# Alex-McAvoy/Light-Graph-Convolutional-Recommendation-Algorithm-based-on-Hybrid-Spreading

Measured on AMD Instinct MI355X. Metric: propagation edges/sec + full-catalog top-K recs/sec, 1/2/4/8 MI355X, higher is better.
Workload: dtype f32; 1 GPU; c5-d64; users=1000000, items=1000000, interactions=100000000, directed_nnz=200000000, dim=64, layers=3, parallelism=row-shard x1 + RCCL all-gather per layer

## Files before the change

include/lgcnhs.h:

```cpp
#ifndef LGCNHS_H
#define LGCNHS_H

#include <stddef.h>
#include <stdint.h>

#ifdef __cplusplus
extern "C" {
#endif

typedef void *lg_stream_t;

enum lg_status {
  LG_OK = 0,
  LG_ERR_ARG = 1,
  LG_ERR_HIP = 2,
  LG_ERR_WORKSPACE = 3,
};

#define LG_ABI_VERSION 16
int lg_abi_version(void);
const char *lg_last_error(void);


int lg_csr_rowptr_from_sorted(const int64_t *keys, int64_t nnz, int64_t n_rows,
                              int64_t *rowptr, lg_stream_t stream);

int lg_gcn_norm_f32(const int64_t *rowptr, int64_t n_nodes, float *dis,
                    lg_stream_t stream);

int lg_gcn_edge_weight_f32(const int64_t *rowptr, const int32_t *src, const float *dis,
                           int64_t n_rows, int64_t row_offset, float *w,
                           lg_stream_t stream);

enum lg_acc_mode {
  LG_ACC_NONE = 0,
  LG_ACC_FIRST = 1,
  LG_ACC_MID = 2,
  LG_ACC_LAST = 3,
  LG_ACC_ONLY = 4,
};
int lg_spmm_layer_f32(const int64_t *rowptr, const int32_t *src, const float *dis,
                      const float *w, const float *x, float *y, const float *x0, float *acc,
// ... 39 lines not shown
                      lg_stream_t stream);
int lg_spmm_long_rows_f16(const int64_t *seg_beg, const int64_t *seg_end,
                          const int32_t *seg_node, int64_t n_seg, const int32_t *long_node,
                          const int64_t *seg_ptr, int64_t n_long, const int32_t *src,
                          const float *dis, const float *w, const void *xh, void *yh,
                          const float *x0, float *acc, float *out, int32_t dim,
                          int32_t acc_mode, float denom, float *partial, lg_stream_t stream);

size_t lg_score_topk_ws_bytes(int64_t n_users, int64_t n_items, int32_t dim, int32_t k,
                              int32_t n_splits);
int lg_score_topk_f32(const float *eu, const float *ei, int64_t n_users, int64_t n_items,
                      int32_t dim, const int64_t *ex_rowptr, const int32_t *ex_col,
                      float mask_value, int32_t k, int32_t n_splits, float *out_val,
                      int64_t *out_idx, void *ws, size_t ws_bytes, lg_stream_t stream);

size_t lg_score_topk_screened_ws_bytes(int64_t n_users, int64_t n_items, int32_t dim,
                                       int32_t k, int32_t n_splits);
int lg_score_topk_screened_f32(const float *eu, const float *ei, const void *eu_bf16,
                               const void *ei_bf16, const float *umarg, int64_t n_users,
                               int64_t n_items, int32_t dim, const int64_t *ex_rowptr,
                               const int32_t *ex_col, float mask_value, int32_t k,
                               int32_t n_splits, float *out_val, int64_t *out_idx, void *ws,
                               size_t ws_bytes, lg_stream_t stream);

int lg_score_dense_f32(const float *eu, const float *ei, int64_t n_users, int64_t n_items,
                       int32_t dim, const int64_t *ex_rowptr, const int32_t *ex_col,
                       float mask_value, float *G, int64_t ldg, lg_stream_t stream);


int lg_spread_general_f64(const int64_t *item_rowptr, const int32_t *item_users,
                          const int64_t *user_rowptr, const int32_t *user_items,
                          int64_t n_users, int64_t n_items, double *gW,
                          lg_stream_t stream);

size_t lg_spread_hybrid_ws_bytes(int64_t n_items, int64_t n_users);
int lg_spread_hybrid_f64(const int64_t *item_rowptr, const int32_t *item_users,
                         const int64_t *user_rowptr, const int32_t *user_items,
                         const double *k_item, int64_t n_users, int64_t n_items, double lambda,
                         double *W, void *ws, size_t ws_bytes, lg_stream_t stream);

int lg_hybrid_weight_f64(const double *gW, const double *k_item, int64_t n_items,
                         double lambda, int32_t transpose_gw, double *W,
                         lg_stream_t stream);

int lg_spread_resource_f64(const int64_t *user_rowptr, const int32_t *user_items,
                           const double *W, int64_t n_users, int64_t n_items, double *F,
// ... 84 lines not shown
```

light-graph-convolutional-recommendation-algorithm-based-on-hybrid-spreading_amd/csrc/topk.hip:

```cpp
#include <stdlib.h>

#include "common.h"

namespace lg {

typedef float f32x4 __attribute__((ext_vector_type(4)));

template <int Q>
__device__ __forceinline__ void load_piece(const float *__restrict__ p, float (&v)[Q]) {
  const float4 *p4 = reinterpret_cast<const float4 *>(p);
#pragma unroll
  for (int t = 0; t < Q / 4; ++t) {
    const float4 q = p4[t];
    v[4 * t + 0] = q.x;
    v[4 * t + 1] = q.y;
    v[4 * t + 2] = q.z;
    v[4 * t + 3] = q.w;
  }
}

typedef float f32x4v __attribute__((ext_vector_type(4)));

typedef unsigned u32x4v __attribute__((ext_vector_type(4)));
template <int D>
// ... 295 lines not shown
#define LG_RING_LA 5
#endif
#ifndef LG_RING_LAG
#define LG_RING_LAG 1
#endif
#ifndef LG_RING2_CAP
#define LG_RING2_CAP 112
#endif
#ifndef LG_RING2_NBUF
#define LG_RING2_NBUF 9
#endif
#ifndef LG_RING4_CAP
#define LG_RING4_CAP 160
#endif
#ifndef LG_RING4_NBUF
#define LG_RING4_NBUF 4
#endif
#ifndef LG_RING4_LA
#define LG_RING4_LA 2
#endif
#ifndef LG_RING4_W
#define LG_RING4_W 8
#endif
#ifndef LG_RING_NG
#define LG_RING_NG 2
#endif
#ifndef LG_RING_W
#define LG_RING_W (16 / LG_RING_NG)
#endif

constexpr int ring_chunk_bytes(int D, int W) {
  if (W == 8 || W == 4) return D >= 64 || W >= 8 ? 8192 : 4096;
  for (int m = 1; m < 64; ++m) {
    const int cb = 1024 * W * m;
    if (cb >= 4096 && (cb / (2 * D)) % 16 == 0) return cb;
  }
  return 0;
}

template <int D, int NG, int WAVES, int M, int CAP, int NBUF, int LA, int LAG, bool SEEDP,
          bool GL = false>
__global__ __launch_bounds__(64 * WAVES) void k_topk_ring(
    const float *__restrict__ eu, const float *__restrict__ ei, const __bf16 *__restrict__ eub,
    const __bf16 *__restrict__ eib, const float *__restrict__ umarg, int64_t n_users,
    int64_t n_items, const int64_t *__restrict__ ex_rowptr,
    const int32_t *__restrict__ ex_col, float mask_value, int k, int n_splits,
    int64_t items_per_split, float *__restrict__ out_val, int64_t *__restrict__ out_idx,
    float *__restrict__ part_val, int32_t *__restrict__ part_idx,
    const float *__restrict__ seed_val, uint2 *__restrict__ gl_list) {
  static_assert(M == 1 || M == 2 || M == 4, "list slabs");
  static_assert(GL ? (CAP <= 64 && CAP > 16) : (CAP <= 64 * M && CAP > 32 * M), "list capacity");
  constexpr int CAPG = 64 * M;
  constexpr int Q = D / 4;
  constexpr int S = D / 32;
  constexpr int CB = ring_chunk_bytes(D, WAVES);
  constexpr int CI = CB / (2 * D), TPC = CI / 16, PR = D / 8, RB = 2 * D;
  constexpr int PPT = CB / 16 / (64 * WAVES);
  static_assert(PPT >= 1 && CI * PR == 64 * WAVES * PPT, "whole DMA pieces per thread");
  static_assert(LAG >= 1 && LA > LAG && NBUF > LA, "ring shape");
  constexpr int TPC_S = TPC < 4 ? TPC : 4;
  constexpr int NCLS = 16 * TPC_S;
  constexpr int R = M == 1 ? (NCLS >= 64 ? 1 : 2) : 4;
  __shared__ uint32_t lk[WAVES][NG][16][SEEDP ? 1 : CAP];
  __shared__ uint16_t lt[WAVES][NG][16][SEEDP ? 1 : CAP];
  __shared__ int exs[WAVES][64];
  __shared__ __attribute__((aligned(16))) char frs[NBUF][CI * RB];
  __shared__ uint32_t prog[WAVES];

  const int wave = threadIdx.x / 64;
  const int lane = lane_id();
  const int ul = lane & 15;
  const int gq = lane >> 4;
  const int64_t tile = blockIdx.x / n_splits;
  const int split = blockIdx.x % n_splits;
  const int64_t ubase = (tile * WAVES + wave) * (16 * NG);
  const int64_t i0 = (int64_t)split * items_per_split;
  int64_t i1 = i0 + items_per_split;
  if (i1 > n_items) i1 = n_items;
  const int n_valid = i1 > i0 ? (int)(i1 - i0) : 0;
  const int n_t = (n_valid + 15) / 16;

  bf16x8 ub[NG][S];
  float marg[NG];
  bool uvalid[NG];
  int64_t ex_pos[NG], ex_hi[NG];
// ... 555 lines not shown
      if constexpr (SEEDP) {
        seed_chunk(c, acc);
        LG_CLK1(9, t_scr);
        continue;
      }
      uint32_t gm = test_chunk(acc);
      LG_CLK1(9, t_scr);
#ifdef LG_SCREEN_PROBE
      asm volatile("" ::"s"(gm));
      gm = 0;
#endif
      if (gm != 0) process_hits(c, acc, gm);
    }
    asm volatile("s_waitcnt vmcnt(0)" ::: "memory");
  }

  wave_sync();
  if constexpr (SEEDP) {
    constexpr int NV = TPC_S * R * 4;
#pragma unroll
    for (int g = 0; g < NG; ++g) {
      const int64_t user = ubase + g * 16 + ul;
      int E = 0;
      if (ex_rowptr && user < n_users) {
        const int64_t e0 = ex_rowptr[user], e1 = ex_rowptr[user + 1];
        E = (int)(lower_bound_i32(ex_col, e0, e1, (int32_t)i1) -
                  lower_bound_i32(ex_col, e0, e1, (int32_t)i0));
      }
      const int need = k + E;
      uint32_t o[NV];
#pragma unroll
      for (int tt = 0; tt < TPC_S; ++tt)
#pragma unroll
        for (int l = 0; l < R; ++l)
#pragma unroll
          for (int r = 0; r < 4; ++r) {
            const float x = cmax[g][tt][l][r];
            o[(tt * R + l) * 4 + r] = ford(x);
          }
      uint32_t T = 0u;
#pragma unroll 1
      for (int b = 31; b >= 0; --b) {
        const uint32_t c = T | (1u << b);
        int n = 0;
#pragma unroll
        for (int j = 0; j < NV; ++j) n += o[j] >= c ? 1 : 0;
        n += __shfl_xor(n, 16);
        n += __shfl_xor(n, 32);
        if (n >= need) T = c;
      }
// ... 243 lines not shown
#endif
#ifndef LG_GL4_NG
#define LG_GL4_NG 1
#endif
#ifndef LG_GL_NG
#define LG_GL_NG 2
#endif
#ifndef LG_TOPK_LDS_LISTS
#define LG_TOPK_LDS_LISTS 0
#endif
static int screen_slab_m(int k) {
  if (LG_TOPK_LDS_LISTS) return 0;
  if (k <= 32) return LG_TOPK_GL32 ? 2 : 0;
  return k <= 64 ? 2 : 4;
}

template <int D>
static void dispatch_topk_screen(int M, bool seedp, const float *eu, const float *ei,
                                 const __bf16 *eub, const __bf16 *eib, const float *umarg,
                                 int64_t n_users, int64_t n_items, const int64_t *ex_rowptr,
                                 const int32_t *ex_col, float mask_value, int k, int n_splits,
                                 int64_t items_per_split, float *out_val, int64_t *out_idx,
                                 float *part_val, int32_t *part_idx, const float *seed_val,
                                 uint2 *gl_list, hipStream_t stream) {
#define LG_RING_LAUNCH(NG, W, MM, CAP, NBUF, LA, LAG, SEEDP, GLM)                             \
  {                                                                                           \
    const int64_t upb = (int64_t)(W) * (NG) * 16;                                             \
    const int64_t tiles = (n_users + upb - 1) / upb;                                          \
    k_topk_ring<D, NG, W, MM, CAP, NBUF, LA, LAG, SEEDP, GLM>                                 \
        <<<dim3((unsigned)(tiles * n_splits)), dim3(64 * (W)), 0, stream>>>(                  \
            eu, ei, eub, eib, umarg, n_users, n_items, ex_rowptr, ex_col, mask_value, k,      \
            n_splits, items_per_split, out_val, out_idx, part_val, part_idx, seed_val,        \
            gl_list);                                                                         \
  }
  const int gm = seedp ? 0 : screen_slab_m(k);
  if (gm == 2) {
    LG_RING_LAUNCH(LG_GL_NG, 8, 2, LG_GL_CAP, LG_GL_NBUF, LG_GL_LA, 1, false, true)
  } else if (gm == 4) {
    LG_RING_LAUNCH((D <= 64 ? LG_GL4_NG : LG_GL_NG), 8, 4, LG_GL_CAP, LG_GL_NBUF, LG_GL_LA, 1,
                   false, true)
  } else if (M == 1 && seedp) {
    LG_RING_LAUNCH(LG_RING_NG, LG_RING_W, 1, LG_RING_CAP, LG_RING_NBUF, LG_RING_LA,
                   LG_RING_LAG, true, false)
  } else if (M == 1) {
    LG_RING_LAUNCH(LG_RING_NG, LG_RING_W, 1, LG_RING_CAP, LG_RING_NBUF, LG_RING_LA,
                   LG_RING_LAG, false, false)
  } else if (M == 2 && seedp) {
    LG_RING_LAUNCH(1, 8, 2, LG_RING2_CAP, LG_RING2_NBUF, LG_RING_LA, LG_RING_LAG, true, false)
  } else if (M == 2) {
    if (LG_TOPK_LDS_LISTS)
      LG_RING_LAUNCH(1, 8, 2, LG_RING2_CAP, LG_RING2_NBUF, LG_RING_LA, LG_RING_LAG, false, false)
  } else if (seedp) {
    LG_RING_LAUNCH(LG_SEED4_NG, 8, 4, 160, LG_SEED4_NBUF, LG_SEED4_LA, 1, true, false)
  } else if constexpr (D > 64) {
    if (LG_TOPK_LDS_LISTS) LG_RING_LAUNCH(1, 8, 4, 160, 4, 2, 1, false, false)
  } else {
// ... 4 lines not shown
}

static int cap_m(int k) { return k <= 32 ? 1 : (k <= 64 ? 2 : 4); }

static size_t screened_part_bytes(int64_t n_users, int k, int ns) {
  return ns > 1 ? (size_t)ns * (size_t)n_users * (size_t)k * (sizeof(float) + sizeof(int32_t))
                : 0;
}
static size_t screened_slab_bytes(int64_t n_users, int k, int ns) {
  return (size_t)ns * (size_t)n_users * 64 * (size_t)screen_slab_m(k) * sizeof(uint2);
}

static int64_t split_len(int64_t n_items, int n_splits) {
  int64_t per = (n_items + n_splits - 1) / n_splits;
  per = (per + 15) / 16 * 16;
  return per < 16 ? 16 : per;
}

static int screened_splits(int64_t n_items, int n_splits) {
  const int64_t need = (n_items + ((int64_t)1 << (kTileBits + 4)) - 1) >> (kTileBits + 4);
  return n_splits > need ? n_splits : (int)need;
}

}

using namespace lg;

extern "C" size_t lg_score_topk_ws_bytes(int64_t n_users, int64_t n_items, int32_t dim,
                                         int32_t k, int32_t n_splits) {
  (void)dim;
  if (n_items > 0 && n_splits >= 1) n_splits = screened_splits(n_items, n_splits);
  if (n_splits <= 1 || n_users <= 0 || k <= 0) return 0;
  return (size_t)n_splits * (size_t)n_users * (size_t)k * (sizeof(float) + sizeof(int32_t));
}

extern "C" size_t lg_score_topk_screened_ws_bytes(int64_t n_users, int64_t n_items,
                                                  int32_t dim, int32_t k, int32_t n_splits) {
  (void)dim;
  if (n_users <= 0 || n_items <= 0 || n_items >= 0x7fffffff || k < 1 || k > 128 ||
      n_splits < 1)
    return 0;
  const int64_t per = split_len(n_items, screened_splits(n_items, n_splits));
  const int ns = (int)((n_items + per - 1) / per);
  return screened_part_bytes(n_users, k, ns) + screened_slab_bytes(n_users, k, ns);
}

// ... 24 lines not shown
    part_val = (float *)ws;
    part_idx = (int32_t *)((char *)ws + (size_t)ns * n_users * k * sizeof(float));
  }
  hipStream_t s = (hipStream_t)stream;
  const int M = cap_m(k);
  if (topk_probe() == 2) ex_rowptr = nullptr, ex_col = nullptr;
  switch (dim) {
    case 32: dispatch_topk<32>(M, eu, ei, n_users, n_items, ex_rowptr, ex_col, mask_value, k, ns, per, out_val, out_idx, part_val, part_idx, s); break;
    case 64: dispatch_topk<64>(M, eu, ei, n_users, n_items, ex_rowptr, ex_col, mask_value, k, ns, per, out_val, out_idx, part_val, part_idx, s); break;
    default: dispatch_topk<128>(M, eu, ei, n_users, n_items, ex_rowptr, ex_col, mask_value, k, ns, per, out_val, out_idx, part_val, part_idx, s); break;
  }
  int st = launch_status("lg_score_topk_f32");
  if (st != LG_OK || ns == 1) return st;
  const unsigned blocks = (unsigned)((n_users + 3) / 4);
  if (k <= 64)
    k_topk_merge<2><<<dim3(blocks), dim3(256), 0, s>>>(part_val, part_idx, n_users, k, ns,
                                                        out_val, out_idx);
  else
    k_topk_merge<4><<<dim3(blocks), dim3(256), 0, s>>>(part_val, part_idx, n_users, k, ns,
                                                        out_val, out_idx);
  return launch_status("lg_score_topk_f32(merge)");
}

extern "C" int lg_score_topk_screened_f32(const float *eu, const float *ei, const void *eu_bf16,
                                          const void *ei_bf16, const float *umarg,
                                          int64_t n_users, int64_t n_items, int32_t dim,
                                          const int64_t *ex_rowptr, const int32_t *ex_col,
                                          float mask_value, int32_t k, int32_t n_splits,
                                          float *out_val, int64_t *out_idx, void *ws,
                                          size_t ws_bytes, lg_stream_t stream) {
  LG_REQUIRE(eu && ei && eu_bf16 && ei_bf16 && umarg && out_val && out_idx,
             "lg_score_topk_screened_f32: null pointer");
  LG_REQUIRE(n_users >= 0 && n_items > 0 && n_items < 0x7fffffff,
             "lg_score_topk_screened_f32: n_items must be in [1, 2^31-1)");
  LG_REQUIRE(dim == 32 || dim == 64 || dim == 128,
             "lg_score_topk_screened_f32: dim %d not in {32,64,128}", dim);
  LG_REQUIRE(k >= 1 && k <= 128, "lg_score_topk_screened_f32: k=%d not in [1,128]", k);
  LG_REQUIRE(n_splits >= 1 && n_splits <= 4096, "lg_score_topk_screened_f32: bad n_splits %d",
             n_splits);
  LG_REQUIRE(!ex_rowptr == !ex_col,
             "lg_score_topk_screened_f32: ex_rowptr/ex_col must both be set");
  LG_REQUIRE(((uintptr_t)eu_bf16 & 15) == 0 && ((uintptr_t)ei_bf16 & 15) == 0,
             "lg_score_topk_screened_f32: bf16 copies must be 16-byte aligned");
  if (n_users == 0) return LG_OK;
  const int64_t per = split_len(n_items, screened_splits(n_items, n_splits));
  const int ns = (int)((n_items + per - 1) / per);
  float *part_val = nullptr;
  int32_t *part_idx = nullptr;
  uint2 *gl_list = nullptr;
  {
    const size_t part = screened_part_bytes(n_users, k, ns);
    const size_t need = part + screened_slab_bytes(n_users, k, ns);
    if (need > 0 && (!ws || ws_bytes < need)) {
      set_error("lg_score_topk_screened_f32: workspace %zu < %zu bytes", ws_bytes, need);
      return LG_ERR_WORKSPACE;
    }
    if (ns > 1) {
      part_val = (float *)ws;
      part_idx = (int32_t *)((char *)ws + (size_t)ns * n_users * k * sizeof(float));
    }
    if (screen_slab_m(k)) gl_list = (uint2 *)((char *)ws + part);
  }
  hipStream_t s = (hipStream_t)stream;
  const int M = cap_m(k);
  const __bf16 *ub = (const __bf16 *)eu_bf16, *ib = (const __bf16 *)ei_bf16;
  auto pass = [&](bool seedp, int64_t n_it, int nsp, int64_t per_sp, const float *seed) {
    switch (dim) {
      case 32: dispatch_topk_screen<32>(M, seedp, eu, ei, ub, ib, umarg, n_users, n_it, ex_rowptr, ex_col, mask_value, k, nsp, per_sp, out_val, out_idx, part_val, part_idx, seed, gl_list, s); break;
      case 64: dispatch_topk_screen<64>(M, seedp, eu, ei, ub, ib, umarg, n_users, n_it, ex_rowptr, ex_col, mask_value, k, nsp, per_sp, out_val, out_idx, part_val, part_idx, seed, gl_list, s); break;
      default: dispatch_topk_screen<128>(M, seedp, eu, ei, ub, ib, umarg, n_users, n_it, ex_rowptr, ex_col, mask_value, k, nsp, per_sp, out_val, out_idx, part_val, part_idx, seed, gl_list, s); break;
    }
    int st = launch_status("lg_score_topk_screened_f32");
    if (st != LG_OK || nsp == 1) return st;
    if (seedp) {
      k_seed_combine<<<dim3((unsigned)((n_users + 255) / 256)), dim3(256), 0, s>>>(
          part_val, n_users, k, nsp, out_val);
      return launch_status("lg_score_topk_screened_f32(seeds)");
    }
    const unsigned blocks = (unsigned)((n_users + 3) / 4);
    if (k <= 64)
      k_topk_merge<2><<<dim3(blocks), dim3(256), 0, s>>>(part_val, part_idx, n_users, k, nsp,
                                                          out_val, out_idx);
    else
      k_topk_merge<4><<<dim3(blocks), dim3(256), 0, s>>>(part_val, part_idx, n_users, k, nsp,
                                                          out_val, out_idx);
    return launch_status("lg_score_topk_screened_f32(merge)");
  };
  const int64_t n_seed = n_items / (k > 32 ? LG_TOPK_SEED_DIV_HI : LG_TOPK_SEED_DIV) / 16 * 16;
  const bool seeded = lg_topk_seeding() && n_seed >= (int64_t)k * 64;
  if (seeded) {
    const int64_t per_s = split_len(n_seed, ns);
    const int ns_s = (int)((n_seed + per_s - 1) / per_s);
    const int st = pass(true, n_seed, ns_s, per_s, nullptr);
    if (st != LG_OK) return st;
  }
  return pass(false, n_items, ns, per, seeded ? out_val : nullptr);
}

extern "C" int lg_score_dense_f32(const float *eu, const float *ei, int64_t n_users,
                                  int64_t n_items, int32_t dim, const int64_t *ex_rowptr,
                                  const int32_t *ex_col, float mask_value, float *G,
                                  int64_t ldg, lg_stream_t stream) {
  LG_REQUIRE(eu && ei && G, "lg_score_dense_f32: null pointer");
  LG_REQUIRE(n_users >= 0 && n_items >= 0 && n_items < 0x7fffffff && ldg >= n_items,
             "lg_score_dense_f32: bad sizes");
  LG_REQUIRE(dim == 32 || dim == 64 || dim == 128, "lg_score_dense_f32: dim %d not in {32,64,128}",
             dim);
  LG_REQUIRE(!ex_rowptr == !ex_col, "lg_score_dense_f32: ex_rowptr/ex_col must both be set");
  if (n_users == 0 || n_items == 0) return LG_OK;
  const int64_t ipb = 1024;
  const int64_t chunks = (n_items + ipb - 1) / ipb;
  const int64_t ugrps = (n_users + 63) / 64;
  hipStream_t s = (hipStream_t)stream;
  dim3 grid((unsigned)(ugrps * chunks)), block(256);
  switch (dim) {
    case 32: k_score_dense<32><<<grid, block, 0, s>>>(eu, ei, n_users, n_items, ex_rowptr, ex_col, mask_value, G, ldg, ipb); break;
    case 64: k_score_dense<64><<<grid, block, 0, s>>>(eu, ei, n_users, n_items, ex_rowptr, ex_col, mask_value, G, ldg, ipb); break;
    default: k_score_dense<128><<<grid, block, 0, s>>>(eu, ei, n_users, n_items, ex_rowptr, ex_col, mask_value, G, ldg, ipb); break;
  }
// ... 13 lines not shown
```

light-graph-convolutional-recommendation-algorithm-based-on-hybrid-spreading_amd/lgcnhs/_native.py:

```python
from __future__ import annotations

import ctypes
import os
import threading

import torch

PKG_DIR = os.path.dirname(os.path.dirname(os.path.abspath(__file__)))
LIB_PATH = os.path.join(PKG_DIR, "lib", "liblgcnhs.so")
LIB_PATH = os.environ.get("LGCNHS_LIB_PATH") or LIB_PATH

LG_OK = 0
LG_ACC_NONE, LG_ACC_FIRST, LG_ACC_MID, LG_ACC_LAST, LG_ACC_ONLY = 0, 1, 2, 3, 4
LG_EXCL_DROP, LG_EXCL_NONE = 0, 1
ABI_VERSION = 16

_vp = ctypes.c_void_p
_i64 = ctypes.c_int64
_i32 = ctypes.c_int32
_f32 = ctypes.c_float
_f64 = ctypes.c_double
_sz = ctypes.c_size_t

SIGNATURES = {
    "lg_abi_version": (ctypes.c_int, []),
    "lg_last_error": (ctypes.c_char_p, []),
    "lg_csr_rowptr_from_sorted": (ctypes.c_int, [_vp, _i64, _i64, _vp, _vp]),
    "lg_gcn_norm_f32": (ctypes.c_int, [_vp, _i64, _vp, _vp]),
    "lg_gcn_edge_weight_f32": (ctypes.c_int, [_vp, _vp, _vp, _i64, _i64, _vp, _vp]),
    "lg_spmm_layer_f32": (
        ctypes.c_int,
        [_vp, _vp, _vp, _vp, _vp, _vp, _vp, _vp, _vp, _i64, _i64, _i32, _i32, _f32, _i64, _vp],
    ),
    "lg_spmm_layer_live_f32": (
        ctypes.c_int,
        [_vp, _vp, _vp, _vp, _vp, _vp, _vp, _vp, _vp, _i64, _i64, _i32, _i32, _f32, _i64, _vp,
         _vp],
    ),
# ... 13 lines not shown
         _f32, _vp, _vp, _vp],
    ),
    "lg_mark_neighbors_u8": (ctypes.c_int, [_vp, _vp, _i64, _vp, _vp, _vp]),
    "lg_rows_f32_to_f16": (ctypes.c_int, [_vp, _i64, _i32, _vp, _vp]),
    "lg_spmm_layer_f16": (
        ctypes.c_int,
        [_vp, _vp, _vp, _vp, _vp, _vp, _vp, _vp, _vp, _i64, _i64, _i32, _i32, _f32, _i64, _vp],
    ),
    "lg_spmm_long_rows_f16": (
        ctypes.c_int,
        [_vp, _vp, _vp, _i64, _vp, _vp, _i64, _vp, _vp, _vp, _vp, _vp, _vp, _vp, _vp, _i32, _i32,
         _f32, _vp, _vp],
    ),
    "lg_score_topk_ws_bytes": (_sz, [_i64, _i64, _i32, _i32, _i32]),
    "lg_score_topk_screened_ws_bytes": (_sz, [_i64, _i64, _i32, _i32, _i32]),
    "lg_score_topk_f32": (
        ctypes.c_int,
        [_vp, _vp, _i64, _i64, _i32, _vp, _vp, _f32, _i32, _i32, _vp, _vp, _vp, _sz, _vp],
    ),
    "lg_score_topk_screened_f32": (
        ctypes.c_int,
        [_vp, _vp, _vp, _vp, _vp, _i64, _i64, _i32, _vp, _vp, _f32, _i32, _i32, _vp, _vp, _vp,
         _sz, _vp],
    ),
    "lg_score_dense_f32": (
        ctypes.c_int,
        [_vp, _vp, _i64, _i64, _i32, _vp, _vp, _f32, _vp, _i64, _vp],
    ),
    "lg_spread_general_f64": (ctypes.c_int, [_vp, _vp, _vp, _vp, _i64, _i64, _vp, _vp]),
    "lg_hybrid_weight_f64": (ctypes.c_int, [_vp, _vp, _i64, _f64, _i32, _vp, _vp]),
    "lg_spread_hybrid_ws_bytes": (_sz, [_i64, _i64]),
    "lg_spread_hybrid_f64": (ctypes.c_int, [_vp, _vp, _vp, _vp, _vp, _i64, _i64, _f64, _vp, _vp,
                                            _sz, _vp]),
    "lg_spread_resource_f64": (ctypes.c_int, [_vp, _vp, _vp, _i64, _i64, _vp, _i64, _vp]),
    "lg_rows_topk_f64": (
        ctypes.c_int,
        [_vp, _i64, _i64, _i64, _vp, _vp, _i32, _vp, _vp, _i32, _i32, _vp, _vp, _vp],
    ),
    "lg_hybrid_recip_f64": (ctypes.c_int, [_vp, _i64, _f64, _vp, _vp, _vp]),
    "lg_inv_degree_f64": (ctypes.c_int, [_vp, _i64, _vp, _vp]),
    "lg_spread_group_cursor": (ctypes.c_int, [_vp, _vp, _vp, _i64, _i32, _i32, _i32, _i32, _vp,
                                              _vp, _vp, _vp, _vp]),
    "lg_spread_group_bound": (ctypes.c_int, [_vp, _vp, _i64, _vp, _i32, _vp, _vp]),
    "lg_spread_group_units": (ctypes.c_int, [_vp, _i64, _i32, _i32, _i32, _i32, _i64, _vp, _vp]),
    "lg_spread_group_rows_ws_bytes": (_sz, [_i64, _i32]),
    "lg_spread_group_rows_f64": (
# ... 116 lines not shown
```

light-graph-convolutional-recommendation-algorithm-based-on-hybrid-spreading_amd/lgcnhs/ops.py:

```python
from __future__ import annotations

import numpy as np
import torch

from . import _native as N
from .graph import Adjacency, RowSets

MASK_VALUE = float(-(1 << 10))


def _f32(t: torch.Tensor, name: str) -> torch.Tensor:
    N.require_gpu(t, name)
    if t.dtype != torch.float32:
        raise TypeError(f"{name} must be float32, got {t.dtype}")
    return t.contiguous()


def run_layer(rowptr, src, dis, w, x, y, x0, acc, out, n_rows: int, row_offset: int,
              mode: int, denom: float, plan=None, live=None, row_mask=None) -> None:
    dim = x.shape[1]
    thr = plan.threshold if (plan is not None and plan.n_long) else 0
    strm = N.stream_handle(x.device)
    half = x.dtype == torch.float16
    if half:
# ... 285 lines not shown
SCREEN_DEFAULT = True
SCREEN_MIN_WORK = {32: 6e8, 128: 1e9}


def screen_pays(n_users: int, n_items: int, k: int) -> bool:
    for kmax, work in SCREEN_MIN_WORK.items():
        if k <= kmax:
            return float(n_users) * float(n_items) >= work
    return False


def screen_margins(un: torch.Tensor, ue: torch.Tensor, inorm: torch.Tensor,
                   ierr: torch.Tensor, dim: int) -> torch.Tensor:
    I = inorm.max().double()
    DI = ierr.max().double()
    u, e = un.double(), ue.double()
    m = (e * I + (u + e) * DI + (2.01 * dim * 2.0 ** -24 + 2.0 ** -22) * u * I) \
        * (1.0 + 2.0 ** -20) + 1e-30
    m32 = m.float()
    return torch.where(m32.double() < m, torch.nextafter(m32, torch.full_like(m32, float("inf"))),
                       m32)


def score_topk(eu: torch.Tensor, ei: torch.Tensor, k: int, excl: RowSets | None = None,
               mask_value: float = MASK_VALUE, n_splits: int | None = None,
               screen: bool | None = None):
    eu, ei = _f32(eu, "eu"), _f32(ei, "ei")
    nu, d = eu.shape
    ni = ei.shape[0]
    if screen is None:
        screen = SCREEN_DEFAULT and screen_pays(nu, ni, k)
    if ei.shape[1] != d:
        raise ValueError("eu/ei dims differ")
    if excl is not None and excl.n_rows != nu:
        raise ValueError(f"exclusion rows {excl.n_rows} != users {nu}")
    ns = (_splits_for(nu, ni, k, _resident_blocks(eu.device, k, screen), screen, d)
          if n_splits is None else int(n_splits))
    ws_fn = (N.lib().lg_score_topk_screened_ws_bytes if screen and nu > 0
             else N.lib().lg_score_topk_ws_bytes)
    ws_bytes = ws_fn(nu, ni, d, k, ns)
    ws = torch.empty(max(ws_bytes, 1), dtype=torch.uint8, device=eu.device)
    val = torch.empty((nu, k), dtype=torch.float32, device=eu.device)
    idx = torch.empty((nu, k), dtype=torch.int64, device=eu.device)
    ex_rp = N.ptr(excl.rowptr if excl else None)
    ex_c = N.ptr(excl.col if excl else None)
    if screen and nu > 0:
        ub, un, ue = bound_operands(eu, with_err=True)
        ib, inorm, ierr = bound_operands(ei, with_err=True)
        umarg = screen_margins(un, ue, inorm, ierr, d)
        N.check(N.lib().lg_score_topk_screened_f32(
            N.ptr(eu), N.ptr(ei), N.ptr(ub), N.ptr(ib), N.ptr(umarg), nu, ni, d, ex_rp, ex_c,
            float(mask_value), int(k), ns, N.ptr(val), N.ptr(idx), N.ptr(ws), ws_bytes,
            N.stream_handle(eu.device)), "lg_score_topk_screened_f32")
        return val, idx
    N.check(N.lib().lg_score_topk_f32(
        N.ptr(eu), N.ptr(ei), nu, ni, d, ex_rp, ex_c, float(mask_value), int(k), ns,
        N.ptr(val), N.ptr(idx), N.ptr(ws), ws_bytes, N.stream_handle(eu.device)),
        "lg_score_topk_f32")
    return val, idx


def score_dense(eu: torch.Tensor, ei: torch.Tensor, excl: RowSets | None = None,
                mask_value: float = MASK_VALUE) -> torch.Tensor:
    eu, ei = _f32(eu, "eu"), _f32(ei, "ei")
    nu, d = eu.shape
    ni = ei.shape[0]
    G = torch.empty((nu, ni), dtype=torch.float32, device=eu.device)
    N.check(N.lib().lg_score_dense_f32(
        N.ptr(eu), N.ptr(ei), nu, ni, d, N.ptr(excl.rowptr if excl else None),
        N.ptr(excl.col if excl else None), float(mask_value), N.ptr(G), ni,
        N.stream_handle(eu.device)), "lg_score_dense_f32")
    return G


class Interactions:

# ... 633 lines not shown
```

Before: 26.91 billion edge-layers/s.

## Seed screened top-K threshold from a high-norm item sample

Adds a radix-select pipeline that picks the highest-norm items (about n_items/16), writes their ids, a membership bitmap and gathered bf16 rows, then runs the seeding pass of the screened top-K over this sample instead of a contiguous item slice. The seeding pass counts exclusions through the bitmap with a wave reduction. The goal is tighter initial thresholds, so the full screened pass processes fewer hits. In exchange it adds several small kernels per call and a bitmap-based exclusion loop.

```diff
diff --git a/include/lgcnhs.h b/include/lgcnhs.h
--- a/include/lgcnhs.h
+++ b/include/lgcnhs.h
@@ -17,7 +17,7 @@
   LG_ERR_WORKSPACE = 3,
 };
 
-#define LG_ABI_VERSION 16
+#define LG_ABI_VERSION 17
 int lg_abi_version(void);
 const char *lg_last_error(void);
 
@@ -103,6 +103,21 @@
                                const int32_t *ex_col, float mask_value, int32_t k,
                                int32_t n_splits, float *out_val, int64_t *out_idx, void *ws,
                                size_t ws_bytes, lg_stream_t stream);
+
+int lg_score_topk_seeded_f32(const float *eu, const float *ei, const void *eu_bf16,
+                             const void *ei_bf16, const float *umarg, int64_t n_users,
+                             int64_t n_items, int32_t dim, const int64_t *ex_rowptr,
+                             const int32_t *ex_col, float mask_value, int32_t k,
+                             int32_t n_splits, const int32_t *sample_ids,
+                             const void *sample_rows, int64_t n_sample,
+                             const uint32_t *sample_bits, float *out_val, int64_t *out_idx,
+                             void *ws, size_t ws_bytes, lg_stream_t stream);
+
+size_t lg_topk_seed_sample_ws_bytes(int64_t n_items, int64_t n_sample);
+int lg_topk_seed_sample_f32(const float *inorm, const void *ei_bf16, int64_t n_items,
+                            int32_t dim, int64_t n_sample, int32_t *sample_ids,
+                            void *sample_rows, uint32_t *sample_bits, void *ws,
+                            size_t ws_bytes, lg_stream_t stream);
 
 int lg_score_dense_f32(const float *eu, const float *ei, int64_t n_users, int64_t n_items,
                        int32_t dim, const int64_t *ex_rowptr, const int32_t *ex_col,
diff --git a/light-graph-convolutional-recommendation-algorithm-based-on-hybrid-spreading_amd/csrc/topk.hip b/light-graph-convolutional-recommendation-algorithm-based-on-hybrid-spreading_amd/csrc/topk.hip
--- a/light-graph-convolutional-recommendation-algorithm-based-on-hybrid-spreading_amd/csrc/topk.hip
+++ b/light-graph-convolutional-recommendation-algorithm-based-on-hybrid-spreading_amd/csrc/topk.hip
@@ -341,6 +341,9 @@
 #ifndef LG_RING4_W
 #define LG_RING4_W 8
 #endif
+#ifndef LG_SEED_R64
+#define LG_SEED_R64 1
+#endif
 #ifndef LG_RING_NG
 #define LG_RING_NG 2
 #endif
@@ -366,7 +369,8 @@
     const int32_t *__restrict__ ex_col, float mask_value, int k, int n_splits,
     int64_t items_per_split, float *__restrict__ out_val, int64_t *__restrict__ out_idx,
     float *__restrict__ part_val, int32_t *__restrict__ part_idx,
-    const float *__restrict__ seed_val, uint2 *__restrict__ gl_list) {
+    const float *__restrict__ seed_val, uint2 *__restrict__ gl_list,
+    const int32_t *__restrict__ samp_ids, const uint32_t *__restrict__ samp_bits) {
   static_assert(M == 1 || M == 2 || M == 4, "list slabs");
   static_assert(GL ? (CAP <= 64 && CAP > 16) : (CAP <= 64 * M && CAP > 32 * M), "list capacity");
   constexpr int CAPG = 64 * M;
@@ -379,7 +383,7 @@
   static_assert(LAG >= 1 && LA > LAG && NBUF > LA, "ring shape");
   constexpr int TPC_S = TPC < 4 ? TPC : 4;
   constexpr int NCLS = 16 * TPC_S;
-  constexpr int R = M == 1 ? (NCLS >= 64 ? 1 : 2) : 4;
+  constexpr int R = M == 1 ? (NCLS >= 64 ? LG_SEED_R64 : 2) : 4;
   __shared__ uint32_t lk[WAVES][NG][16][SEEDP ? 1 : CAP];
   __shared__ uint16_t lt[WAVES][NG][16][SEEDP ? 1 : CAP];
   __shared__ int exs[WAVES][64];
@@ -981,10 +985,29 @@
     for (int g = 0; g < NG; ++g) {
       const int64_t user = ubase + g * 16 + ul;
       int E = 0;
-      if (ex_rowptr && user < n_users) {
+      if (ex_rowptr && user < n_users && n_valid > 0) {
         const int64_t e0 = ex_rowptr[user], e1 = ex_rowptr[user + 1];
-        E = (int)(lower_bound_i32(ex_col, e0, e1, (int32_t)i1) -
-                  lower_bound_i32(ex_col, e0, e1, (int32_t)i0));
+        if (samp_bits) {
+          const int32_t id_lo = samp_ids[i0], id_hi = samp_ids[i1 - 1];
+          for (int64_t e = e0 + gq; e < e1; e += 32) {
+            int32_t x[8];
+#pragma unroll
+            for (int j = 0; j < 8; ++j) x[j] = e + 4 * j < e1 ? ex_col[e + 4 * j] : -1;
+#pragma unroll
+            for (int j = 0; j < 8; ++j) {
+              const bool in = x[j] >= id_lo && x[j] <= id_hi;
+              const uint32_t xc = (uint32_t)(in ? x[j] : id_lo);
+              E += in ? (int)((samp_bits[xc >> 5] >> (xc & 31u)) & 1u) : 0;
+            }
+          }
+        } else {
+          E = (int)(lower_bound_i32(ex_col, e0, e1, (int32_t)i1) -
+                    lower_bound_i32(ex_col, e0, e1, (int32_t)i0));
+        }
+      }
+      if (samp_bits) {
+        E += __shfl_xor(E, 16);
+        E += __shfl_xor(E, 32);
       }
       const int need = k + E;
       uint32_t o[NV];
@@ -1274,7 +1297,8 @@
                                  const int32_t *ex_col, float mask_value, int k, int n_splits,
                                  int64_t items_per_split, float *out_val, int64_t *out_idx,
                                  float *part_val, int32_t *part_idx, const float *seed_val,
-                                 uint2 *gl_list, hipStream_t stream) {
+                                 uint2 *gl_list, const int32_t *samp_ids,
+                                 const uint32_t *samp_bits, hipStream_t stream) {
 #define LG_RING_LAUNCH(NG, W, MM, CAP, NBUF, LA, LAG, SEEDP, GLM)                             \
   {                                                                                           \
     const int64_t upb = (int64_t)(W) * (NG) * 16;                                             \
@@ -1283,7 +1307,7 @@
         <<<dim3((unsigned)(tiles * n_splits)), dim3(64 * (W)), 0, stream>>>(                  \
             eu, ei, eub, eib, umarg, n_users, n_items, ex_rowptr, ex_col, mask_value, k,      \
             n_splits, items_per_split, out_val, out_idx, part_val, part_idx, seed_val,        \
-            gl_list);                                                                         \
+            gl_list, samp_ids, samp_bits);                                                    \
   }
   const int gm = seedp ? 0 : screen_slab_m(k);
   if (gm == 2) {
@@ -1334,6 +1358,159 @@
   return n_splits > need ? n_splits : (int)need;
 }
 
+constexpr int kSelBlocks = 1024;
+constexpr int kSelHist = 0, kSelGt = 1024, kSelEq = kSelGt + kSelBlocks,
+              kSelT = kSelEq + kSelBlocks, kSelWords = kSelT + 2;
+
+__device__ __forceinline__ uint32_t norm_key(float x) {
+  if (x != x) return 0u;
+  return ford(x == 0.f ? 0.f : x);
+}
+
+__device__ __forceinline__ void sel_resolve(const uint32_t *hist, int np, uint32_t n_sample,
+                                            uint32_t &prefix, uint32_t &rank) {
+  __shared__ uint32_t sc[256];
+  __shared__ uint32_t s_bin, s_rank;
+  const int t = threadIdx.x;
+  prefix = 0u;
+  rank = n_sample;
+  for (int p = 0; p < np; ++p) {
+    const uint32_t v = hist[256 * p + t];
+    sc[t] = v;
+    __syncthreads();
+    for (int s = 1; s < 256; s <<= 1) {
+      const uint32_t a = t + s < 256 ? sc[t + s] : 0u;
+      __syncthreads();
+      sc[t] += a;
+      __syncthreads();
+    }
+    const uint32_t incl = sc[t], above_t = incl - v;
+    if (above_t < rank && rank <= incl) {
+      s_bin = (uint32_t)t;
+      s_rank = rank - above_t;
+    }
+    __syncthreads();
+    prefix = (prefix << 8) | s_bin;
+    rank = s_rank;
+    __syncthreads();
+  }
+}
+
+__global__ __launch_bounds__(256) void k_sel_hist(const float *__restrict__ inorm,
+                                                  int64_t n_items, uint32_t n_sample, int p,
+                                                  uint32_t *__restrict__ ws) {
+  __shared__ uint32_t lh[256];
+  uint32_t prefix, rank;
+  sel_resolve(ws + kSelHist, p, n_sample, prefix, rank);
+  lh[threadIdx.x] = 0u;
+  __syncthreads();
+  const int sh = 24 - 8 * p;
+  const int64_t stride = (int64_t)gridDim.x * 256;
+  for (int64_t base = (int64_t)blockIdx.x * 256; base < n_items; base += stride) {
+    const int64_t i = base + threadIdx.x;
+    const uint32_t key = i < n_items ? norm_key(inorm[i]) : 0u;
+    const bool m = i < n_items && (uint32_t)((uint64_t)key >> (sh + 8)) == prefix;
+    const uint32_t bin = (key >> sh) & 255u;
+    const uint64_t bm = __ballot(m);
+    if (bm == 0) continue;
+    const uint32_t b0 = (uint32_t)__shfl((int)bin, __builtin_ctzll(bm));
+    if (__ballot(m && bin == b0) == bm) {
+      if (lane_id() == __builtin_ctzll(bm)) atomicAdd(&lh[b0], (uint32_t)__popcll(bm));
+    } else if (m) {
+      atomicAdd(&lh[bin], 1u);
+    }
+  }
+  __syncthreads();
+  if (lh[threadIdx.x]) atomicAdd(&ws[kSelHist + 256 * p + threadIdx.x], lh[threadIdx.x]);
+}
+
+__global__ __launch_bounds__(256) void k_sel_count(const float *__restrict__ inorm,
+                                                   int64_t n_items, uint32_t n_sample,
+                                                   int64_t ipb, uint32_t *__restrict__ ws) {
+  __shared__ uint32_t c_gt, c_eq;
+  uint32_t T, take;
+  sel_resolve(ws + kSelHist, 4, n_sample, T, take);
+  if (threadIdx.x == 0) c_gt = 0u, c_eq = 0u;
+  __syncthreads();
+  const int64_t i0 = (int64_t)blockIdx.x * ipb;
+  const int64_t i1 = i0 + ipb < n_items ? i0 + ipb : n_items;
+  uint32_t gt = 0u, eq = 0u;
+  for (int64_t i = i0 + threadIdx.x; i < i1; i += 256) {
+    const uint32_t key = norm_key(inorm[i]);
+    gt += key > T ? 1u : 0u;
+    eq += key == T ? 1u : 0u;
+  }
+  if (gt) atomicAdd(&c_gt, gt);
+  if (eq) atomicAdd(&c_eq, eq);
+  __syncthreads();
+  if (threadIdx.x == 0) {
+    ws[kSelGt + blockIdx.x] = c_gt;
+    ws[kSelEq + blockIdx.x] = c_eq;
+    if (blockIdx.x == 0) ws[kSelT] = T, ws[kSelT + 1] = take;
+  }
+}
+
+__global__ __launch_bounds__(256) void k_sel_write(const float *__restrict__ inorm,
+                                                   int64_t n_items, int64_t ipb,
+                                                   const uint32_t *__restrict__ ws,
+                                                   int32_t *__restrict__ sample_ids,
+                                                   uint32_t *__restrict__ bits) {
+  __shared__ uint32_t r_gt, r_eq;
+  __shared__ uint32_t w_gt[4], w_eq[4];
+  const int t = threadIdx.x, wave = t / 64, lane = lane_id();
+  const uint32_t T = ws[kSelT], take = ws[kSelT + 1];
+  if (t == 0) r_gt = 0u, r_eq = 0u;
+  __syncthreads();
+  {
+    uint32_t a = 0u, b = 0u;
+    for (int j = t; j < (int)blockIdx.x; j += 256) a += ws[kSelGt + j], b += ws[kSelEq + j];
+    if (a) atomicAdd(&r_gt, a);
+    if (b) atomicAdd(&r_eq, b);
+  }
+  __syncthreads();
+  uint32_t gt_run = r_gt, eq_run = r_eq;
+  const int64_t n_words = (n_items + 31) / 32;
+  const int64_t i0 = (int64_t)blockIdx.x * ipb;
+  const int64_t i1 = i0 + ipb < n_items ? i0 + ipb : n_items;
+  for (int64_t base = i0; base < i1; base += 256) {
+    const int64_t i = base + t;
+    const uint32_t key = i < i1 ? norm_key(inorm[i]) : 0u;
+    const bool gt = i < i1 && key > T, eq = i < i1 && key == T;
+    const uint64_t bgt = __ballot(gt), beq = __ballot(eq);
+    if (lane == 0) w_gt[wave] = (uint32_t)__popcll(bgt), w_eq[wave] = (uint32_t)__popcll(beq);
+    __syncthreads();
+    uint32_t g = gt_run + (uint32_t)__popcll(bgt & lanemask_lt());
+    uint32_t e = eq_run + (uint32_t)__popcll(beq & lanemask_lt());
+    for (int w = 0; w < 4; ++w) {
+      if (w < wave) g += w_gt[w], e += w_eq[w];
+      gt_run += w_gt[w];
+      eq_run += w_eq[w];
+    }
+    const bool sel = gt || (eq && e < take);
+    if (sel) sample_ids[g + (e < take ? e : take)] = (int32_t)i;
+    const uint64_t bs = __ballot(sel);
+    const int64_t w0 = (base + 64 * wave) >> 5;
+    if (lane == 0 && w0 < n_words) bits[w0] = (uint32_t)bs;
+    if (lane == 1 && w0 + 1 < n_words) bits[w0 + 1] = (uint32_t)(bs >> 32);
+    __syncthreads();
+  }
+}
+
+__global__ __launch_bounds__(256) void k_sel_gather(const uint4 *__restrict__ eib,
+                                                    const int32_t *__restrict__ ids,
+                                                    int64_t n_sample, int PR,
+                                                    uint4 *__restrict__ rows) {
+  const int64_t p = (int64_t)blockIdx.x * 256 + threadIdx.x;
+  const int64_t r = p / PR;
+  if (r >= n_sample) return;
+  rows[p] = eib[(int64_t)ids[r] * PR + (p - r * PR)];
+}
+
+static int64_t sel_items_per_block(int64_t n_items) {
+  const int64_t per = (n_items + kSelBlocks - 1) / kSelBlocks;
+  return (per + 255) / 256 * 256;
+}
+
 }
 
 using namespace lg;
@@ -1404,26 +1581,37 @@
   return launch_status("lg_score_topk_f32(merge)");
 }
 
-extern "C" int lg_score_topk_screened_f32(const float *eu, const float *ei, const void *eu_bf16,
-                                          const void *ei_bf16, const float *umarg,
-                                          int64_t n_users, int64_t n_items, int32_t dim,
-                                          const int64_t *ex_rowptr, const int32_t *ex_col,
-                                          float mask_value, int32_t k, int32_t n_splits,
-                                          float *out_val, int64_t *out_idx, void *ws,
-                                          size_t ws_bytes, lg_stream_t stream) {
+static int score_topk_screened(const char *fn, const float *eu, const float *ei,
+                               const void *eu_bf16, const void *ei_bf16, const float *umarg,
+                               int64_t n_users, int64_t n_items, int32_t dim,
+                               const int64_t *ex_rowptr, const int32_t *ex_col,
+                               float mask_value, int32_t k, int32_t n_splits,
+                               const int32_t *sample_ids, const void *sample_rows,
+                               int64_t n_sample, const uint32_t *sample_bits, float *out_val,
+                               int64_t *out_idx, void *ws, size_t ws_bytes,
+                               lg_stream_t stream) {
   LG_REQUIRE(eu && ei && eu_bf16 && ei_bf16 && umarg && out_val && out_idx,
-             "lg_score_topk_screened_f32: null pointer");
+             "%s: null pointer", fn);
   LG_REQUIRE(n_users >= 0 && n_items > 0 && n_items < 0x7fffffff,
-             "lg_score_topk_screened_f32: n_items must be in [1, 2^31-1)");
-  LG_REQUIRE(dim == 32 || dim == 64 || dim == 128,
-             "lg_score_topk_screened_f32: dim %d not in {32,64,128}", dim);
-  LG_REQUIRE(k >= 1 && k <= 128, "lg_score_topk_screened_f32: k=%d not in [1,128]", k);
-  LG_REQUIRE(n_splits >= 1 && n_splits <= 4096, "lg_score_topk_screened_f32: bad n_splits %d",
-             n_splits);
-  LG_REQUIRE(!ex_rowptr == !ex_col,
-             "lg_score_topk_screened_f32: ex_rowptr/ex_col must both be set");
+             "%s: n_items must be in [1, 2^31-1)", fn);
+  LG_REQUIRE(dim == 32 || dim == 64 || dim == 128, "%s: dim %d not in {32,64,128}", fn, dim);
+  LG_REQUIRE(k >= 1 && k <= 128, "%s: k=%d not in [1,128]", fn, k);
+  LG_REQUIRE(n_splits >= 1 && n_splits <= 4096, "%s: bad n_splits %d", fn, n_splits);
+  LG_REQUIRE(!ex_rowptr == !ex_col, "%s: ex_rowptr/ex_col must both be set", fn);
   LG_REQUIRE(((uintptr_t)eu_bf16 & 15) == 0 && ((uintptr_t)ei_bf16 & 15) == 0,
-             "lg_score_topk_screened_f32: bf16 copies must be 16-byte aligned");
+             "%s: bf16 copies must be 16-byte aligned", fn);
+  const bool sampled = sample_ids || sample_rows || sample_bits || n_sample != 0;
+  if (sampled) {
+    LG_REQUIRE(sample_ids && sample_rows && sample_bits,
+               "%s: null pointer (sample_ids / sample_rows / sample_bits: all or none)", fn);
+    LG_REQUIRE(n_sample >= 16 && n_sample <= n_items && n_sample % 16 == 0,
+               "%s: n_sample=%lld must be a multiple of 16 in [16, n_items]", fn,
+               (long long)n_sample);
+    LG_REQUIRE(((uintptr_t)sample_rows & 15) == 0, "%s: sample_rows must be 16-byte aligned",
+               fn);
+    LG_REQUIRE(((uintptr_t)sample_ids & 3) == 0 && ((uintptr_t)sample_bits & 3) == 0,
+               "%s: sample_ids / sample_bits must be 4-byte aligned", fn);
+  }
   if (n_users == 0) return LG_OK;
   const int64_t per = split_len(n_items, screened_splits(n_items, n_splits));
   const int ns = (int)((n_items + per - 1) / per);
@@ -1434,7 +1622,7 @@
     const size_t part = screened_part_bytes(n_users, k, ns);
     const size_t need = part + screened_slab_bytes(n_users, k, ns);
     if (need > 0 && (!ws || ws_bytes < need)) {
-      set_error("lg_score_topk_screened_f32: workspace %zu < %zu bytes", ws_bytes, need);
+      set_error("%s: workspace %zu < %zu bytes", fn, ws_bytes, need);
       return LG_ERR_WORKSPACE;
     }
     if (ns > 1) {
@@ -1446,18 +1634,20 @@
   hipStream_t s = (hipStream_t)stream;
   const int M = cap_m(k);
   const __bf16 *ub = (const __bf16 *)eu_bf16, *ib = (const __bf16 *)ei_bf16;
+  const int32_t *samp_ids = nullptr;
+  const uint32_t *samp_bits = nullptr;
   auto pass = [&](bool seedp, int64_t n_it, int nsp, int64_t per_sp, const float *seed) {
     switch (dim) {
-      case 32: dispatch_topk_screen<32>(M, seedp, eu, ei, ub, ib, umarg, n_users, n_it, ex_rowptr, ex_col, mask_value, k, nsp, per_sp, out_val, out_idx, part_val, part_idx, seed, gl_list, s); break;
-      case 64: dispatch_topk_screen<64>(M, seedp, eu, ei, ub, ib, umarg, n_users, n_it, ex_rowptr, ex_col, mask_value, k, nsp, per_sp, out_val, out_idx, part_val, part_idx, seed, gl_list, s); break;
-      default: dispatch_topk_screen<128>(M, seedp, eu, ei, ub, ib, umarg, n_users, n_it, ex_rowptr, ex_col, mask_value, k, nsp, per_sp, out_val, out_idx, part_val, part_idx, seed, gl_list, s); break;
-    }
-    int st = launch_status("lg_score_topk_screened_f32");
+      case 32: dispatch_topk_screen<32>(M, seedp, eu, ei, ub, ib, umarg, n_users, n_it, ex_rowptr, ex_col, mask_value, k, nsp, per_sp, out_val, out_idx, part_val, part_idx, seed, gl_list, samp_ids, samp_bits, s); break;
+      case 64: dispatch_topk_screen<64>(M, seedp, eu, ei, ub, ib, umarg, n_users, n_it, ex_rowptr, ex_col, mask_value, k, nsp, per_sp, out_val, out_idx, part_val, part_idx, seed, gl_list, samp_ids, samp_bits, s); break;
+      default: dispatch_topk_screen<128>(M, seedp, eu, ei, ub, ib, umarg, n_users, n_it, ex_rowptr, ex_col, mask_value, k, nsp, per_sp, out_val, out_idx, part_val, part_idx, seed, gl_list, samp_ids, samp_bits, s); break;
+    }
+    int st = launch_status(fn);
     if (st != LG_OK || nsp == 1) return st;
     if (seedp) {
       k_seed_combine<<<dim3((unsigned)((n_users + 255) / 256)), dim3(256), 0, s>>>(
           part_val, n_users, k, nsp, out_val);
-      return launch_status("lg_score_topk_screened_f32(seeds)");
+      return launch_status(fn);
     }
     const unsigned blocks = (unsigned)((n_users + 3) / 4);
     if (k <= 64)
@@ -1466,17 +1656,104 @@
     else
       k_topk_merge<4><<<dim3(blocks), dim3(256), 0, s>>>(part_val, part_idx, n_users, k, nsp,
                                                           out_val, out_idx);
-    return launch_status("lg_score_topk_screened_f32(merge)");
+    return launch_status(fn);
   };
-  const int64_t n_seed = n_items / (k > 32 ? LG_TOPK_SEED_DIV_HI : LG_TOPK_SEED_DIV) / 16 * 16;
+  const int64_t n_seed =
+      sampled ? n_sample
+              : n_items / (k > 32 ? LG_TOPK_SEED_DIV_HI : LG_TOPK_SEED_DIV) / 16 * 16;
   const bool seeded = lg_topk_seeding() && n_seed >= (int64_t)k * 64;
   if (seeded) {
     const int64_t per_s = split_len(n_seed, ns);
     const int ns_s = (int)((n_seed + per_s - 1) / per_s);
+    if (sampled) {
+      ib = (const __bf16 *)sample_rows;
+      samp_ids = sample_ids;
+      samp_bits = sample_bits;
+    }
     const int st = pass(true, n_seed, ns_s, per_s, nullptr);
+    ib = (const __bf16 *)ei_bf16;
+    samp_ids = nullptr;
+    samp_bits = nullptr;
     if (st != LG_OK) return st;
   }
   return pass(false, n_items, ns, per, seeded ? out_val : nullptr);
+}
+
+extern "C" int lg_score_topk_screened_f32(const float *eu, const float *ei, const void *eu_bf16,
+                                          const void *ei_bf16, const float *umarg,
+                                          int64_t n_users, int64_t n_items, int32_t dim,
+                                          const int64_t *ex_rowptr, const int32_t *ex_col,
+                                          float mask_value, int32_t k, int32_t n_splits,
+                                          float *out_val, int64_t *out_idx, void *ws,
+                                          size_t ws_bytes, lg_stream_t stream) {
+  return score_topk_screened("lg_score_topk_screened_f32", eu, ei, eu_bf16, ei_bf16, umarg,
+                             n_users, n_items, dim, ex_rowptr, ex_col, mask_value, k, n_splits,
+                             nullptr, nullptr, 0, nullptr, out_val, out_idx, ws, ws_bytes,
+                             stream);
+}
+
+extern "C" int lg_score_topk_seeded_f32(const float *eu, const float *ei, const void *eu_bf16,
+                                        const void *ei_bf16, const float *umarg,
+                                        int64_t n_users, int64_t n_items, int32_t dim,
+                                        const int64_t *ex_rowptr, const int32_t *ex_col,
+                                        float mask_value, int32_t k, int32_t n_splits,
+                                        const int32_t *sample_ids, const void *sample_rows,
+                                        int64_t n_sample, const uint32_t *sample_bits,
+                                        float *out_val, int64_t *out_idx, void *ws,
+                                        size_t ws_bytes, lg_stream_t stream) {
+  return score_topk_screened("lg_score_topk_seeded_f32", eu, ei, eu_bf16, ei_bf16, umarg,
+                             n_users, n_items, dim, ex_rowptr, ex_col, mask_value, k, n_splits,
+                             sample_ids, sample_rows, n_sample, sample_bits, out_val, out_idx,
+                             ws, ws_bytes, stream);
+}
+
+extern "C" size_t lg_topk_seed_sample_ws_bytes(int64_t n_items, int64_t n_sample) {
+  if (n_items <= 0 || n_items >= 0x7fffffff || n_sample <= 0 || n_sample > n_items) return 0;
+  return (size_t)kSelWords * sizeof(uint32_t);
+}
+
+extern "C" int lg_topk_seed_sample_f32(const float *inorm, const void *ei_bf16,
+                                       int64_t n_items, int32_t dim, int64_t n_sample,
+                                       int32_t *sample_ids, void *sample_rows,
+                                       uint32_t *sample_bits, void *ws, size_t ws_bytes,
+                                       lg_stream_t stream) {
+  LG_REQUIRE(inorm && ei_bf16 && sample_ids && sample_rows && sample_bits && ws,
+             "lg_topk_seed_sample_f32: null pointer");
+  LG_REQUIRE(n_items > 0 && n_items < 0x7fffffff,
+             "lg_topk_seed_sample_f32: n_items must be in [1, 2^31-1)");
+  LG_REQUIRE(dim == 32 || dim == 64 || dim == 128,
+             "lg_topk_seed_sample_f32: dim %d not in {32,64,128}", dim);
+  LG_REQUIRE(n_sample >= 16 && n_sample <= n_items && n_sample % 16 == 0,
+             "lg_topk_seed_sample_f32: n_sample=%lld must be a multiple of 16 in [16, n_items]",
+             (long long)n_sample);
+  LG_REQUIRE(((uintptr_t)ei_bf16 & 15) == 0 && ((uintptr_t)sample_rows & 15) == 0,
+             "lg_topk_seed_sample_f32: ei_bf16 / sample_rows must be 16-byte aligned");
+  LG_REQUIRE(((uintptr_t)inorm & 3) == 0 && ((uintptr_t)sample_ids & 3) == 0 &&
+                 ((uintptr_t)sample_bits & 3) == 0 && ((uintptr_t)ws & 3) == 0,
+             "lg_topk_seed_sample_f32: inorm / sample_ids / sample_bits / ws must be 4-byte "
+             "aligned");
+  const size_t need = lg_topk_seed_sample_ws_bytes(n_items, n_sample);
+  if (ws_bytes < need) {
+    set_error("lg_topk_seed_sample_f32: workspace %zu < %zu bytes", ws_bytes, need);
+    return LG_ERR_WORKSPACE;
+  }
+  hipStream_t s = (hipStream_t)stream;
+  uint32_t *w = (uint32_t *)ws;
+  if (hipMemsetAsync(w + kSelHist, 0, 4 * 256 * sizeof(uint32_t), s) != hipSuccess)
+    return launch_status("lg_topk_seed_sample_f32");
+  const int64_t ipb = sel_items_per_block(n_items);
+  const unsigned nb = (unsigned)((n_items + ipb - 1) / ipb);
+  const int64_t hb = (n_items + 255) / 256;
+  const unsigned nh = (unsigned)(hb < kSelBlocks ? hb : kSelBlocks);
+  for (int p = 0; p < 4; ++p)
+    k_sel_hist<<<dim3(nh), dim3(256), 0, s>>>(inorm, n_items, (uint32_t)n_sample, p, w);
+  k_sel_count<<<dim3(nb), dim3(256), 0, s>>>(inorm, n_items, (uint32_t)n_sample, ipb, w);
+  k_sel_write<<<dim3(nb), dim3(256), 0, s>>>(inorm, n_items, ipb, w, sample_ids, sample_bits);
+  const int PR = dim / 8;
+  const int64_t pieces = n_sample * PR;
+  k_sel_gather<<<dim3((unsigned)((pieces + 255) / 256)), dim3(256), 0, s>>>(
+      (const uint4 *)ei_bf16, sample_ids, n_sample, PR, (uint4 *)sample_rows);
+  return launch_status("lg_topk_seed_sample_f32");
 }
 
 extern "C" int lg_score_dense_f32(const float *eu, const float *ei, int64_t n_users,
diff --git a/light-graph-convolutional-recommendation-algorithm-based-on-hybrid-spreading_amd/lgcnhs/_native.py b/light-graph-convolutional-recommendation-algorithm-based-on-hybrid-spreading_amd/lgcnhs/_native.py
--- a/light-graph-convolutional-recommendation-algorithm-based-on-hybrid-spreading_amd/lgcnhs/_native.py
+++ b/light-graph-convolutional-recommendation-algorithm-based-on-hybrid-spreading_amd/lgcnhs/_native.py
@@ -13,7 +13,7 @@
 LG_OK = 0
 LG_ACC_NONE, LG_ACC_FIRST, LG_ACC_MID, LG_ACC_LAST, LG_ACC_ONLY = 0, 1, 2, 3, 4
 LG_EXCL_DROP, LG_EXCL_NONE = 0, 1
-ABI_VERSION = 16
+ABI_VERSION = 17
 
 _vp = ctypes.c_void_p
 _i64 = ctypes.c_int64
@@ -73,6 +73,16 @@
         ctypes.c_int,
         [_vp, _vp, _vp, _vp, _vp, _i64, _i64, _i32, _vp, _vp, _f32, _i32, _i32, _vp, _vp, _vp,
          _sz, _vp],
+    ),
+    "lg_score_topk_seeded_f32": (
+        ctypes.c_int,
+        [_vp, _vp, _vp, _vp, _vp, _i64, _i64, _i32, _vp, _vp, _f32, _i32, _i32, _vp, _vp, _i64,
+         _vp, _vp, _vp, _vp, _sz, _vp],
+    ),
+    "lg_topk_seed_sample_ws_bytes": (_sz, [_i64, _i64]),
+    "lg_topk_seed_sample_f32": (
+        ctypes.c_int,
+        [_vp, _vp, _i64, _i32, _i64, _vp, _vp, _vp, _vp, _sz, _vp],
     ),
     "lg_score_dense_f32": (
         ctypes.c_int,
diff --git a/light-graph-convolutional-recommendation-algorithm-based-on-hybrid-spreading_amd/lgcnhs/ops.py b/light-graph-convolutional-recommendation-algorithm-based-on-hybrid-spreading_amd/lgcnhs/ops.py
--- a/light-graph-convolutional-recommendation-algorithm-based-on-hybrid-spreading_amd/lgcnhs/ops.py
+++ b/light-graph-convolutional-recommendation-algorithm-based-on-hybrid-spreading_amd/lgcnhs/ops.py
@@ -331,6 +331,25 @@
                        m32)
 
 
+def seed_sample_size(n_items: int, k: int) -> int:
+    n = n_items // 16 // 16 * 16
+    return n if n >= 64 * k else 0
+
+
+def seed_sample(ib: torch.Tensor, inorm: torch.Tensor, n_sample: int):
+    ni, d = ib.shape
+    dev = ib.device
+    ids = torch.empty(n_sample, dtype=torch.int32, device=dev)
+    rows = torch.empty((n_sample, d), dtype=torch.int16, device=dev)
+    bits = torch.empty((ni + 31) // 32, dtype=torch.int32, device=dev)
+    ws_bytes = N.lib().lg_topk_seed_sample_ws_bytes(ni, n_sample)
+    ws = torch.empty(max(ws_bytes, 1), dtype=torch.uint8, device=dev)
+    N.check(N.lib().lg_topk_seed_sample_f32(
+        N.ptr(inorm), N.ptr(ib), ni, d, int(n_sample), N.ptr(ids), N.ptr(rows), N.ptr(bits),
+        N.ptr(ws), ws_bytes, N.stream_handle(dev)), "lg_topk_seed_sample_f32")
+    return ids, rows, bits
+
+
 def score_topk(eu: torch.Tensor, ei: torch.Tensor, k: int, excl: RowSets | None = None,
                mask_value: float = MASK_VALUE, n_splits: int | None = None,
                screen: bool | None = None):
@@ -357,10 +376,13 @@
         ub, un, ue = bound_operands(eu, with_err=True)
         ib, inorm, ierr = bound_operands(ei, with_err=True)
         umarg = screen_margins(un, ue, inorm, ierr, d)
-        N.check(N.lib().lg_score_topk_screened_f32(
+        n_sample = seed_sample_size(ni, k)
+        sids, srows, sbits = seed_sample(ib, inorm, n_sample) if n_sample else (None,) * 3
+        N.check(N.lib().lg_score_topk_seeded_f32(
             N.ptr(eu), N.ptr(ei), N.ptr(ub), N.ptr(ib), N.ptr(umarg), nu, ni, d, ex_rp, ex_c,
-            float(mask_value), int(k), ns, N.ptr(val), N.ptr(idx), N.ptr(ws), ws_bytes,
-            N.stream_handle(eu.device)), "lg_score_topk_screened_f32")
+            float(mask_value), int(k), ns, N.ptr(sids), N.ptr(srows), n_sample, N.ptr(sbits),
+            N.ptr(val), N.ptr(idx), N.ptr(ws), ws_bytes, N.stream_handle(eu.device)),
+            "lg_score_topk_seeded_f32")
         return val, idx
     N.check(N.lib().lg_score_topk_f32(
         N.ptr(eu), N.ptr(ei), nu, ni, d, ex_rp, ex_c, float(mask_value), int(k), ns,
```

New measurement: 26.92 billion edge-layers/s (median of 2 runs). No clear change (+0.0%).
